# MarineRoboticsGroup/mac

Hardware: AMD Instinct MI355X
Metric: frank_wolfe_iters_per_sec (higher is better)
Workload: dtype f64; 1 GPU; configs[3]: ER N=100000 ~2M candidates, chain fixed, K=10%; N=100000, m_candidates=2001737, K=200173, fixed_edges=99999, fw_iters=209, parallelism=single GPU

## Files before the change

### include/machip.h

```cpp
#ifndef MACHIP_H
#define MACHIP_H

#include <stdint.h>

#ifdef __cplusplus
extern "C" {
#endif

#define MACHIP_ABI_VERSION 19

typedef enum machip_status {
    MACHIP_OK = 0,
    MACHIP_NOT_CONVERGED = 1,
    MACHIP_DISCONNECTED = 2,
    MACHIP_BAD_ARG = 3,
    MACHIP_HIP_ERROR = 4,
    MACHIP_RCCL_ERROR = 5,
    MACHIP_NO_DEVICE = 6
} machip_status;

typedef struct machip_problem machip_problem;

typedef struct machip_solve_stats {
    int64_t lanczos_steps;
    int64_t spmv_total;
    int64_t vec_passes;
    int64_t restarts;
    int64_t nnz;
    int64_t support;
    double residual;
    double lnorm;
    double gpu_ms;
    double step_ms;
    int64_t steps_timed;
    int64_t steps_lowp;
    double drift;
} machip_solve_stats;

int machip_version(void);
int machip_sizeof_stats(void);
int machip_device_count(void);
const char* machip_last_error(void);

int machip_create(int device, int64_t n,
                  int64_t n_fixed, const int32_t* fi, const int32_t* fj, const double* fw,
                  int64_t m, const int32_t* ci, const int32_t* cj, const double* cw,
                  double min_selection_weight_tol, machip_problem** out);
void machip_destroy(machip_problem* p);

int machip_set_x(machip_problem* p, const double* x);
int machip_get_x(machip_problem* p, double* x);

int machip_assemble(machip_problem* p, int64_t* nnz_out);
int machip_get_laplacian(machip_problem* p, int32_t* indptr, int32_t* indices, double* data);

int machip_fiedler(machip_problem* p, double tol, int max_steps, const double* x0, int warm_start,
                   double* lambda2, double* v_out, double* X_out, int q,
                   machip_solve_stats* stats);

int machip_lowest_pairs(machip_problem* p, int q, double tol, int max_steps, const double* X0, int warm_start,
                        double* lambda_out, double* V_out, double* residual_out, int32_t* steps_out, int32_t* restarts_out,
                        int32_t* status_out, int32_t* reordered_out, int32_t* first_rank_out);
int machip_lowest_pairs_csr(int device, int64_t n, const int32_t* indptr, const int32_t* indices, const double* data,
                            int q, double tol, int max_steps, const double* X0, int warm_start,
                            double* lambda_out, double* V_out, double* residual_out, int32_t* steps_out, int32_t* restarts_out,
                            int32_t* status_out, int32_t* reordered_out, int32_t* first_rank_out);
int machip_lowest_pairs_time(machip_problem* p, int q, double* ms_out);
int machip_gradient_block(machip_problem* p, int q, const double* V, double* G_out);

int machip_set_start(machip_problem* p, const double* x0);

int machip_gradient(machip_problem* p, double* g_out);

int machip_lp_topk(machip_problem* p, int64_t k, double* s_out);

int machip_fw_step(machip_problem* p, int64_t k, int iter, double tol, int max_steps, int warm_start,
                   double* f, double* dual, double* gnorm, machip_solve_stats* stats);
int machip_fw_commit(machip_problem* p);
int machip_fw_run(machip_problem* p, int64_t k, int first_iter, int max_iters, double gap_tol, double grad_tol, double tol,
                  int max_steps, int warm_start, double* upper_inout, double* f_traj, double* dual_traj, double* gnorm_traj,
                  machip_solve_stats* stats, int* modes, int* iters_done);

int machip_round_nearest(machip_problem* p, int64_t k, int decimals, double* rounded_out);

int machip_fiedler_csr(int device, int64_t n, const int32_t* indptr, const int32_t* indices,
                       const double* data, double tol, int max_steps, const double* x0,
// ... 102 lines not shown
```

### mac_amd/_lib.py

```python
from __future__ import annotations

import ctypes as C
import os

import numpy as np

_HERE = os.path.dirname(os.path.abspath(__file__))
LIB_PATH = os.environ.get("MACHIP_LIB") or os.path.join(_HERE, "libmachip.so")

OK, NOT_CONVERGED, DISCONNECTED, BAD_ARG, HIP_ERROR, RCCL_ERROR, NO_DEVICE = range(7)
STATUS_NAMES = ["OK", "NOT_CONVERGED", "DISCONNECTED", "BAD_ARG", "HIP_ERROR", "RCCL_ERROR", "NO_DEVICE"]


class MachipError(RuntimeError):
    def __init__(self, status, msg):
        super().__init__(f"libmachip: {STATUS_NAMES[status] if 0 <= status < 7 else status}: {msg}")
        self.status = status


class NotConverged(MachipError):
    pass


class Disconnected(MachipError):
    """lambda_2 ~ 0 (the reference fails with SuperLU 'Factor is exactly singular')."""


class SolveStats(C.Structure):
    _fields_ = [("lanczos_steps", C.c_int64), ("spmv_total", C.c_int64), ("vec_passes", C.c_int64),
                ("restarts", C.c_int64), ("nnz", C.c_int64), ("support", C.c_int64),
                ("residual", C.c_double), ("lnorm", C.c_double), ("gpu_ms", C.c_double),
                ("step_ms", C.c_double), ("steps_timed", C.c_int64), ("steps_lowp", C.c_int64), ("drift", C.c_double)]

    def asdict(self):
        return {k: getattr(self, k) for k, _ in self._fields_}


_i32p = C.POINTER(C.c_int32)
_f64p = C.POINTER(C.c_double)
_lib = None

_PAIRS_TAIL = [_f64p, _f64p, _f64p, _i32p, _i32p, _i32p, C.POINTER(C.c_int32), C.POINTER(C.c_int32)]
PAIRS_CHUNK = 16

SIGNATURES = {
    "machip_version": (C.c_int, []),
    "machip_sizeof_stats": (C.c_int, []),
    "machip_device_count": (C.c_int, []),
    "machip_last_error": (C.c_char_p, []),
    "machip_create": (C.c_int, [C.c_int, C.c_int64, C.c_int64, _i32p, _i32p, _f64p, C.c_int64, _i32p, _i32p,
                                _f64p, C.c_double, C.POINTER(C.c_void_p)]),
    "machip_destroy": (None, [C.c_void_p]),
    "machip_set_x": (C.c_int, [C.c_void_p, _f64p]),
    "machip_get_x": (C.c_int, [C.c_void_p, _f64p]),
    "machip_assemble": (C.c_int, [C.c_void_p, C.POINTER(C.c_int64)]),
    "machip_get_laplacian": (C.c_int, [C.c_void_p, _i32p, _i32p, _f64p]),
    "machip_fiedler": (C.c_int, [C.c_void_p, C.c_double, C.c_int, _f64p, C.c_int, _f64p, _f64p, _f64p, C.c_int,
                                 C.POINTER(SolveStats)]),
    "machip_lowest_pairs": (C.c_int, [C.c_void_p, C.c_int, C.c_double, C.c_int, _f64p, C.c_int] + _PAIRS_TAIL),
    "machip_lowest_pairs_csr": (C.c_int, [C.c_int, C.c_int64, _i32p, _i32p, _f64p, C.c_int, C.c_double, C.c_int, _f64p, C.c_int] + _PAIRS_TAIL),
    "machip_lowest_pairs_time": (C.c_int, [C.c_void_p, C.c_int, _f64p]),
    "machip_gradient_block": (C.c_int, [C.c_void_p, C.c_int, _f64p, _f64p]),
    "machip_set_start": (C.c_int, [C.c_void_p, _f64p]),
    "machip_gradient": (C.c_int, [C.c_void_p, _f64p]),
    "machip_lp_topk": (C.c_int, [C.c_void_p, C.c_int64, _f64p]),
    "machip_fw_step": (C.c_int, [C.c_void_p, C.c_int64, C.c_int, C.c_double, C.c_int, C.c_int, _f64p, _f64p,
                                 _f64p, C.POINTER(SolveStats)]),
    "machip_fw_commit": (C.c_int, [C.c_void_p]),
    "machip_fw_run": (C.c_int, [C.c_void_p, C.c_int64, C.c_int, C.c_int, C.c_double, C.c_double, C.c_double, C.c_int, C.c_int, _f64p, _f64p,
                                _f64p, _f64p, C.POINTER(SolveStats), C.POINTER(C.c_int), C.POINTER(C.c_int)]),
    "machip_round_nearest": (C.c_int, [C.c_void_p, C.c_int64, C.c_int, _f64p]),
    "machip_fiedler_csr": (C.c_int, [C.c_int, C.c_int64, _i32p, _i32p, _f64p, C.c_double, C.c_int, _f64p, _f64p,
                                     _f64p, _f64p, C.c_int, C.POINTER(SolveStats)]),
    "machip_spmv": (C.c_int, [C.c_void_p, _f64p, _f64p, C.c_int]),
    "machip_landscape": (C.c_int, [C.c_void_p, C.c_int, _f64p]),
    "machip_profile_spmv": (C.c_int, [C.c_void_p, C.c_int, _f64p, _f64p]),
    "machip_comm_unique_id": (C.c_int, [C.c_void_p]),
    "machip_comm_init": (C.c_int, [C.c_void_p, C.c_int, C.c_int, C.c_void_p]),
    "machip_comm_init_local": (C.c_int, [C.POINTER(C.c_void_p), C.c_int]),
    "machip_selftest_watchdog": (C.c_int, [C.c_int, C.c_int]),
    "machip_peer_access": (C.c_int, [C.c_int, C.c_int]),
    "machip_ipc_blob_bytes": (C.c_int, []),
    "machip_ipc_export": (C.c_int, [C.c_void_p, C.c_void_p, C.c_int]),
    "machip_comm_init_ipc": (C.c_int, [C.c_void_p, C.c_int, C.c_int, C.c_void_p, C.c_double]),
    "machip_comm_close_ipc": (C.c_int, [C.c_void_p]),
    "machip_comm_mode": (C.c_int, [C.c_void_p]),
    "machip_shard_plan": (C.c_int, [C.c_int64, C.c_int, C.c_int, C.POINTER(C.c_int64), C.POINTER(C.c_int64), C.POINTER(C.c_int64)]),
    "machip_eval_batch": (C.c_int, [C.c_void_p, C.c_int, _f64p, C.c_double, C.c_int, _f64p, C.POINTER(C.c_int)]),
# ... 169 lines not shown
        h = C.c_void_p()
        check(lib.machip_create(int(device), self.n, len(fw), p_i32(fi), p_i32(fj), p_f64(fw), self.m,
                                p_i32(ci), p_i32(cj), p_f64(cw), float(min_selection_weight_tol), C.byref(h)))
        self._h = h
        self._lib = lib
        self.stats = SolveStats()

    def close(self):
        if getattr(self, "_h", None):
            self._lib.machip_destroy(self._h)
            self._h = None

    def __del__(self):
        try:
            self.close()
        except Exception:
            pass

    def set_x(self, x):
        x = f64(x)
        assert x.shape == (self.m,)
        check(self._lib.machip_set_x(self._h, p_f64(x)))

    def get_x(self):
        x = np.empty(self.m)
        check(self._lib.machip_get_x(self._h, p_f64(x)))
        return x

    def assemble(self):
        nnz = C.c_int64()
        check(self._lib.machip_assemble(self._h, C.byref(nnz)))
        return int(nnz.value)

    def laplacian_csr(self):
        nnz = self.assemble()
        indptr = np.empty(self.n + 1, dtype=np.int32)
        indices = np.empty(nnz, dtype=np.int32)
        data = np.empty(nnz)
        check(self._lib.machip_get_laplacian(self._h, p_i32(indptr), p_i32(indices), p_f64(data)))
        return indptr, indices, data

    def spmv(self, v, variant=0):
        v = f64(v)
        y = np.empty(self.n)
        check(self._lib.machip_spmv(self._h, p_f64(v), p_f64(y), int(variant)))
        return y

    def landscape(self, sweeps=3):
        u = np.empty(self.n)
        check(self._lib.machip_landscape(self._h, int(sweeps), p_f64(u)))
        return u

    def fiedler(self, tol=1e-8, max_steps=0, x0=None, warm_start=False, want_vec=True, q=0):
        lam = C.c_double()
        v = np.empty(self.n) if want_vec else None
        X = np.empty((q, self.n)) if q else None
        x0a = f64(x0) if x0 is not None else None
        st = self._lib.machip_fiedler(self._h, float(tol), int(max_steps), p_f64(x0a), int(bool(warm_start)),
                                      C.byref(lam), p_f64(v), p_f64(X), int(q), C.byref(self.stats))
        check(st)
        return lam.value, v, (X.T if X is not None else None)

    def lowest_pairs(self, q=4, tol=1e-8, max_steps=0, X0=None, warm_start=False, raise_on_cap=False):
        X0 = None if X0 is None else np.asfortranarray(X0, dtype=np.float64)
        assert X0 is None or X0.shape == (self.n, q)
        return _pairs_call(lambda *tail: self._lib.machip_lowest_pairs(self._h, int(q), float(tol), int(max_steps), p_f64(X0),
# ... 500 lines not shown
```

### mac_amd/csrc/kernels.h

```cpp
#pragma once
#include <algorithm>

#include "common.h"

namespace machip {

template <typename T>
struct CsrViewT {
    int n;
    const int* rowptr;
    const int* col;
    const T* val;
};
using CsrView = CsrViewT<double>;

struct PatternView {
    int n;
    const int* prow;
    const int* pcol;
    const int* pk;
    const double* pw;
};

struct LanState {
// ... 42 lines not shown
        const int b = P.prow[r], e = P.prow[r + 1];
        int c = 0, sc = 0;
        for (int p = b + lane; p < e; p += G) {
            const int k = P.pk[p];
            const bool cand = k >= 0;
            const bool act = cand ? x_bit(xbits, k) : true;
            c += act;
            sc += (cand && act);
        }
        c = group_sum_i<G>(c);
        sc = group_sum_i<G>(sc);
        if (lane == 0) {
            cnt[r] = c + 1;
            local += c + 1;
            supp += sc;
            mx = max(mx, c + 1);
        }
    }
    const int tot = block_sum_i(local, sm);
    const int stot = block_sum_i(supp, sm);
#pragma unroll
    for (int o = 32; o > 0; o >>= 1) mx = max(mx, __shfl_xor(mx, o, kWave));
    __syncthreads();
    if ((threadIdx.x & 63) == 0) sm[threadIdx.x >> 6] = mx;
    __syncthreads();
    if (threadIdx.x == 0) {
        blk_sum[blockIdx.x] = tot;
        blk_sum[kAsmGrid + blockIdx.x] = stot;
        const int longest = max(max(sm[0], sm[1]), max(sm[2], sm[3]));
        blk_sum[2 * kAsmGrid + blockIdx.x] = longest;
        if (hsum) {
            hsum[blockIdx.x] = tot; hsum[kAsmGrid + blockIdx.x] = stot; hsum[2 * kAsmGrid + blockIdx.x] = longest;
        }
    }
}

struct PanSpec {
    int NP = 0;
    int C = 1;
    int band = 0;
    int* ps = nullptr;
    double* bd = nullptr;
    int* bpk = nullptr;
    int* ovf = nullptr;
};

template <int G>
__global__ __launch_bounds__(kBlock) void k_asm_fill(PatternView P, const unsigned int* __restrict__ xbits, const double* __restrict__ x,
                                                     int rows_per_block,
                                                     const int* __restrict__ cnt,
                                                     const int* __restrict__ blk_sum,
                                                     int* __restrict__ rowptr, int* __restrict__ col,
                                                     double* __restrict__ val,
                                                     double* __restrict__ blk_lnorm, PanSpec S = PanSpec()) {
    extern __shared__ __attribute__((aligned(16))) char smem_raw[];
    int* s_off = reinterpret_cast<int*>(smem_raw);
    __shared__ int sm_i[4];
    __shared__ double sm_d[4];
    __shared__ int s_chunk[kBlock];
    constexpr int GPB = kBlock / G;
    const int tid = threadIdx.x;
    const int lane = tid % G, g = tid / G;
    const int r0 = blockIdx.x * rows_per_block;
    const int r1 = min(P.n, r0 + rows_per_block);
    const int nr = max(0, r1 - r0);

// ... 1144 lines not shown
        st->prefix = s_prefix; st->kk = need; st->cnt_eq = eq; st->T = T; st->k = k;
        for (int i = 0; i < 7; ++i) st->ticket[i] = 0;
        st->ticket[7] = (unsigned int)s_done;
    }
    if (k <= 0) { if (tid == 0) st->tie_limit = prefer_high ? 0x7fffffffffffffffll : -1; return; }
    if (need >= eq) { if (tid == 0) st->tie_limit = prefer_high ? -1 : 0x7fffffffffffffffll; return; }
    long long runs = 0;
    for (long base = 0; base < m; base += 1024) {
        const long ii = base + tid;
        const long i = prefer_high ? m - 1 - ii : ii;
        const bool is = ii < m && f64_key(g[i]) == T;
        const unsigned long long bal = __ballot(is);
        __syncthreads();
        if (ln == 0) s_cnt[wv] = __popcll(bal);
        __syncthreads();
        int before = 0, tot = 0;
        for (int q = 0; q < 16; ++q) { if (q < wv) before += s_cnt[q]; tot += s_cnt[q]; }
        if (runs + tot >= need) {
            const int rank = before + __popcll(bal & ((1ull << ln) - 1ull));
            if (is && runs + rank + 1 == need) s_found = i;
            __syncthreads();
            if (tid == 0) st->tie_limit = s_found;
            return;
        }
        runs += tot;
    }
    if (tid == 0) st->tie_limit = prefer_high ? -1 : 0x7fffffffffffffffll;
}

__global__ __launch_bounds__(kBlock) void k_fw_final(const double* __restrict__ g, const double* __restrict__ x,
                                                     long m, const SelState* __restrict__ st, double gamma,
                                                     double* __restrict__ x_next, double* __restrict__ s_out,
                                                     double* __restrict__ part ,
                                                     double tol = 0.0, unsigned long long* __restrict__ xbits_next = nullptr) {
#pragma clang fp contract(off)
    __shared__ double sm[4];
    const unsigned long long T = st->T;
    const long long lim = st->tie_limit;
    const bool none = st->k <= 0;
    double d = 0.0, q = 0.0;
    for (long i = (long)blockIdx.x * kBlock + threadIdx.x; i < m; i += (long)gridDim.x * kBlock) {
        const double gi = g[i];
        const unsigned long long key = f64_key(gi);
        const double s = (!none && (key > T || (key == T && (long long)i <= lim))) ? 1.0 : 0.0;
        if (s_out) s_out[i] = s;
        if (x) {
            const double xi = x[i];
            const double diff = s - xi;
            d += gi * diff;
            q += gi * gi;
            if (x_next) {
                const double step = gamma * diff;
                const double xn = xi + step;
                x_next[i] = xn;
                if (xbits_next) {
                    const unsigned long long bal = __ballot(xn > tol);
                    if ((threadIdx.x & 63) == 0) xbits_next[i >> 6] = bal;
                }
            }
        }
    }
    d = block_sum(d, sm);
    q = block_sum(q, sm);
    if (threadIdx.x == 0) { part[blockIdx.x] = d; part[kMaxGrid + blockIdx.x] = q; }
}

__global__ __launch_bounds__(kBlock) void k_round_keys(const double* __restrict__ x, long m, double f,
                                                       double* __restrict__ r) {
#pragma clang fp contract(off)
    for (long i = (long)blockIdx.x * kBlock + threadIdx.x; i < m; i += (long)gridDim.x * kBlock) {
        const double t = x[i] * f;
        r[i] = rint(t) / f;
    }
}
__global__ __launch_bounds__(kBlock) void k_tie_keys(const double* __restrict__ r, const double* __restrict__ cw,
                                                     long m, const SelState* __restrict__ st1,
                                                     double* __restrict__ keys2) {
    const unsigned long long T = st1->T;
    for (long i = (long)blockIdx.x * kBlock + threadIdx.x; i < m; i += (long)gridDim.x * kBlock)
        keys2[i] = f64_key(r[i]) == T ? cw[i] : -__builtin_huge_val();
}
__global__ __launch_bounds__(kBlock) void k_round_mark(const double* __restrict__ r, const double* __restrict__ keys2,
                                                       long m, const SelState* __restrict__ st1,
                                                       const SelState* __restrict__ st2, int two_level,
                                                       double* __restrict__ out) {
    const unsigned long long T1 = st1->T;
    const bool none = st1->k <= 0;
    for (long i = (long)blockIdx.x * kBlock + threadIdx.x; i < m; i += (long)gridDim.x * kBlock) {
        const unsigned long long k1 = f64_key(r[i]);
        bool sel = false;
// ... 63 lines not shown
```

### mac_amd/csrc/mac.h

```cpp
#pragma once
#include <rccl/rccl.h>

#include <algorithm>
#include <cmath>
#include <condition_variable>
#include <memory>

#include "solver.h"

struct machip_problem;

namespace machip {

inline bool completed(int st) { return st == MACHIP_OK || st == MACHIP_NOT_CONVERGED || st == MACHIP_DISCONNECTED; }

struct LocalGroup {
    int nranks = 0;
    std::vector<double*> g;
    std::vector<machip_problem*> members;
    ShardGroup sg;
    bool shard_eig = false;
    int lead_status = MACHIP_OK;
    double lead_lam = 0.0;
    machip_solve_stats lead_stats{};
// ... 11 lines not shown
        std::unique_lock<std::mutex> lk(mu);
        if (broken) return false;
        const unsigned long gen = generation;
        if (++waiting == nranks) { waiting = 0; ++generation; cv.notify_all(); return true; }
        cv.wait(lk, [&] { return generation != gen || broken; });
        return !broken;
    }
    void abort() {
        std::lock_guard<std::mutex> lk(mu);
        broken = true;
        cv.notify_all();
    }
};

}

struct machip_problem {
    int device = 0;
    hipStream_t stream = nullptr;
    int n = 0;
    long m = 0, m_pad = 0;
    double tol_sel = 1e-10;
    int *prow = nullptr, *pcol = nullptr, *pk = nullptr;
    double* pw = nullptr;
    long P = 0;
    int asm_G = 16, asm_rpb = 1, asm_grid = 1;
    int *ci = nullptr, *cj = nullptr;
    double* cw = nullptr;
    double *x = nullptr, *x_next = nullptr, *g = nullptr, *s = nullptr, *scratch_m = nullptr;
    int *cnt = nullptr, *blk_sum = nullptr, *rowptr = nullptr, *col = nullptr;
    double *val = nullptr, *blk_lnorm = nullptr;
    unsigned long long *xb = nullptr, *xb_next = nullptr;
    bool xb_valid = false, xb_next_valid = false;
    long nnz = 0, support = 0;
    int maxlen = 0;
    double lnorm = 0.0;
    bool assembled = false, have_vec = false, csr_only = false;
    bool band_dups_ok = true;
    unsigned int* hist = nullptr;
    machip::SelState* sel = nullptr;
    double* part_fw = nullptr;
    int* h_int = nullptr;
    double* h_dbl = nullptr;
    int* d_hint = nullptr;
    double* d_hdbl = nullptr;
    machip::Solver sol;
    ncclComm_t comm = nullptr;
    std::shared_ptr<machip::LocalGroup> lgroup;
    bool first_collective_pending = false;
    hipEvent_t ev_g0 = nullptr, ev_g1 = nullptr, ev_g2 = nullptr;
    bool ev_g_valid = false;
    std::unique_ptr<machip::IpcGroup> ipcg;
    int rank = 0, nranks = 1;
    bool is_lane = false, lane_fw_ready = false;
    std::vector<machip_problem*> lanes;
    unsigned long start_version = 0;
    unsigned long seen_start_version = ~0ul;

    machip::CsrView csr() const { return machip::CsrView{n, rowptr, col, val}; }
    machip::PatternView pattern() const { return machip::PatternView{n, prow, pcol, pk, pw}; }
};

namespace machip {

inline std::mutex g_csr_mu;
inline machip_problem* g_csr_cache = nullptr;

struct Slot { int col, k; double w; };

inline int build_pattern(machip_problem* p, int64_t nf, const int32_t* fi, const int32_t* fj, const double* fw,
                         int64_t m, const int32_t* ci, const int32_t* cj, const double* cw) {
    const Options& opt = p->sol.opt;
    const int n = p->n;
    std::vector<long> deg((size_t)n + 1, 0);
    auto chk = [&](int a, int b) { return a >= 0 && a < n && b >= 0 && b < n; };
    for (int64_t e = 0; e < nf; ++e) {
        if (!chk(fi[e], fj[e])) return fail(MACHIP_BAD_ARG, "fixed edge endpoint out of range");
        if (fi[e] != fj[e]) { deg[(size_t)fi[e]]++; deg[(size_t)fj[e]]++; }
    }
    for (int64_t e = 0; e < m; ++e) {
        if (!chk(ci[e], cj[e])) return fail(MACHIP_BAD_ARG, "candidate edge endpoint out of range");
        if (ci[e] != cj[e]) { deg[(size_t)ci[e]]++; deg[(size_t)cj[e]]++; }
    }
    std::vector<long> off((size_t)n + 1, 0);
    for (int r = 0; r < n; ++r) off[(size_t)r + 1] = off[(size_t)r] + deg[(size_t)r];
    std::vector<Slot> slots((size_t)off[(size_t)n]);
    std::vector<long> cur(off.begin(), off.end() - 1);
    for (int64_t e = 0; e < nf; ++e) {
        const int a = fi[e], b = fj[e];
        if (a == b) continue;
        slots[(size_t)cur[(size_t)a]++] = Slot{b, -1, fw[e]};
        slots[(size_t)cur[(size_t)b]++] = Slot{a, -1, fw[e]};
    }
    for (int64_t e = 0; e < m; ++e) {
        const int a = ci[e], b = cj[e];
        if (a == b) continue;
        slots[(size_t)cur[(size_t)a]++] = Slot{b, (int)e, cw[e]};
        slots[(size_t)cur[(size_t)b]++] = Slot{a, (int)e, cw[e]};
    }
    std::vector<int> prow((size_t)n + 1, 0);
    std::vector<int> pcol, pk;
    std::vector<double> pw;
    pcol.reserve(slots.size()); pk.reserve(slots.size()); pw.reserve(slots.size());
    for (int r = 0; r < n; ++r) {
        Slot* b = slots.data() + off[(size_t)r];
        Slot* e = slots.data() + off[(size_t)r + 1];
        std::sort(b, e, [](const Slot& x, const Slot& y) {
            if (x.col != y.col) return x.col < y.col;
            return x.k < y.k;
        });
        for (Slot* q = b; q < e; ++q) {
            if (q->k < 0 && !pcol.empty() && (long)pcol.size() > prow[(size_t)r] && pcol.back() == q->col &&
                pk.back() < 0) {
                pw.back() += q->w;
            } else {
                pcol.push_back(q->col); pk.push_back(q->k); pw.push_back(q->w);
            }
        }
        if (pcol.size() > 2000000000ull) return fail(MACHIP_BAD_ARG, "pattern exceeds int32 indexing");
        {
            int band_slots = 0;
            for (size_t q = (size_t)prow[(size_t)r]; q < pcol.size(); ++q) band_slots += (pcol[q] == r - 1 || pcol[q] == r + 1);
            if (band_slots > 7) p->band_dups_ok = false;
        }
        prow[(size_t)r + 1] = (int)pcol.size();
    }
    p->P = (long)pcol.size();
    ST_TRY(dev_alloc(&p->prow, (size_t)n + 1));
    ST_TRY(dev_alloc(&p->pcol, (size_t)p->P)); ST_TRY(dev_alloc(&p->pk, (size_t)p->P)); ST_TRY(dev_alloc(&p->pw, (size_t)p->P));
    HIP_TRY(hipMemcpyAsync(p->prow, prow.data(), sizeof(int) * ((size_t)n + 1), hipMemcpyHostToDevice, p->stream));
    if (p->P) {
        HIP_TRY(hipMemcpyAsync(p->pcol, pcol.data(), sizeof(int) * (size_t)p->P, hipMemcpyHostToDevice, p->stream));
        HIP_TRY(hipMemcpyAsync(p->pk, pk.data(), sizeof(int) * (size_t)p->P, hipMemcpyHostToDevice, p->stream));
        HIP_TRY(hipMemcpyAsync(p->pw, pw.data(), sizeof(double) * (size_t)p->P, hipMemcpyHostToDevice, p->stream));
    }
    HIP_TRY(hipStreamSynchronize(p->stream));
    const double mean = n ? (double)p->P / n : 1.0;
    int G = 4;
    while (G < 64 && G < mean * 0.75) G <<= 1;
    p->asm_G = OPT(asm_g, G);
    const int gpb = kBlock / p->asm_G;
    long nblk = std::min<long>(std::min(kAsmGrid, std::max(1, OPT(asm_maxgrid, kAsmGrid))), ((long)n + gpb - 1) / gpb);
    if (nblk < 1) nblk = 1;
    long rpb = ((long)n + nblk - 1) / nblk;
    rpb = (rpb + gpb - 1) / gpb * gpb;
    p->asm_rpb = (int)rpb;
    p->asm_grid = (int)(((long)n + rpb - 1) / rpb);
    if (p->asm_grid < 1) p->asm_grid = 1;
    if ((rpb + 1) * (long)sizeof(int) > 64 * 1024)
        return fail(MACHIP_BAD_ARG, "num_nodes above the supported 16.7 million (row-offset scan of the assembly kernel)");
    return MACHIP_OK;
}

template <int G>
void launch_asm(machip_problem* p, const PanSpec& S) {
    const PatternView P = p->pattern();
    const unsigned int* xb32 = reinterpret_cast<const unsigned int*>(p->xb);
    k_asm_count<G><<<p->asm_grid, kBlock, 0, p->stream>>>(P, xb32, p->asm_rpb, p->cnt, p->blk_sum, p->d_hint);
    const size_t lds = sizeof(int) * ((size_t)p->asm_rpb + 1);
    k_asm_fill<G><<<p->asm_grid, kBlock, lds, p->stream>>>(P, xb32, p->x, p->asm_rpb, p->cnt, p->blk_sum,
                                                           p->rowptr, p->col, p->val, p->d_hdbl, S);
}

inline int assemble(machip_problem* p) {
    if (p->csr_only) return fail(MACHIP_BAD_ARG, "handle wraps a caller CSR; nothing to assemble");
    PanSpec S;
    ST_TRY(p->sol.pan_spec_prepare(&S));
    if (!p->xb_valid) {
        const int grid = std::max(1, (int)std::min<long>(kMaxGrid, (p->m + kBlock - 1) / kBlock));
        k_x_bits<<<grid, kBlock, 0, p->stream>>>(p->x, p->m, p->tol_sel, p->xb);
        p->xb_valid = true;
    }
    switch (p->asm_G) {
        case 4: launch_asm<4>(p, S); break;
        case 8: launch_asm<8>(p, S); break;
        case 16: launch_asm<16>(p, S); break;
        case 32: launch_asm<32>(p, S); break;
        default: launch_asm<64>(p, S); break;
    }
    HIP_TRY(hipGetLastError());
    const int gb = p->asm_grid;
    HIP_TRY(hipStreamSynchronize(p->stream));
    long nnz = 0, supp = 0;
    int maxlen = 0;
    double ln = 0.0;
    for (int b = 0; b < gb; ++b) {
        nnz += p->h_int[b]; supp += p->h_int[kAsmGrid + b]; maxlen = std::max(maxlen, p->h_int[2 * kAsmGrid + b]);
        ln = std::max(ln, p->h_dbl[b]);
    }
    p->nnz = nnz; p->support = supp / 2; p->lnorm = ln; p->maxlen = maxlen;
    p->assembled = true;
    return MACHIP_OK;
}

inline int alloc_common(machip_problem* p, int vbudget_mb = 0) {
    ST_TRY(p->sol.init(p->n, p->stream, vbudget_mb));
    HIP_TRY(hipHostMalloc((void**)&p->h_int, sizeof(int) * 3 * kAsmGrid, hipHostMallocMapped));
    HIP_TRY(hipHostMalloc((void**)&p->h_dbl, sizeof(double) * std::max(4 * kMaxGrid, kAsmGrid), hipHostMallocMapped));
    HIP_TRY(hipHostGetDevicePointer((void**)&p->d_hint, p->h_int, 0));
    HIP_TRY(hipHostGetDevicePointer((void**)&p->d_hdbl, p->h_dbl, 0));
    return MACHIP_OK;
}

inline int alloc_assembly(machip_problem* p) {
    const size_t cap = (size_t)p->P + (size_t)p->n + 8;
    ST_TRY(dev_alloc(&p->cnt, (size_t)p->n + 1)); ST_TRY(dev_alloc(&p->blk_sum, 3 * kAsmGrid));
    ST_TRY(dev_alloc(&p->rowptr, (size_t)p->n + 1)); ST_TRY(dev_alloc(&p->col, cap)); ST_TRY(dev_alloc(&p->val, cap));
    ST_TRY(dev_alloc(&p->blk_lnorm, kAsmGrid));
    ST_TRY(dev_alloc(&p->xb, (size_t)p->m / 64 + 2)); ST_TRY(dev_alloc(&p->xb_next, (size_t)p->m / 64 + 2));
    p->sol.csr_cap = cap;
    return MACHIP_OK;
}

inline int alloc_fw(machip_problem* p) {
    const size_t mp = (size_t)p->m + 64 * 8;
    if (!p->x_next) ST_TRY(dev_alloc(&p->x_next, mp));
    if (!p->g) ST_TRY(dev_alloc(&p->g, mp));
    if (!p->s) ST_TRY(dev_alloc(&p->s, mp));
    return MACHIP_OK;
}
inline int alloc_fw_select(machip_problem* p) {
    if (!p->hist) ST_TRY(dev_alloc(&p->hist, (6 + kSelRep) * kBins));
    if (!p->sel) ST_TRY(dev_alloc(&p->sel, 2));
    if (!p->part_fw) ST_TRY(dev_alloc(&p->part_fw, 2 * kMaxGrid));
// ... 22 lines not shown
        HIP_TRY(hipStreamSynchronize(p->stream));
        p->sol.have_start = true;
        ++p->start_version;
    }
    machip_solve_stats local;
    memset(&local, 0, sizeof(local));
    p->sol.maxlen_hint = p->maxlen;
    p->sol.support_hint = (p->csr_only && !p->sol.chain_like) ? -1 : p->support;
    p->sol.start_guess = x0 != nullptr;
    const int st = p->sol.solve(p->csr(), p->nnz, p->lnorm, tol, max_steps, (x0 == nullptr && warm_start) ? 1 : 0,
                                kAuto, lambda2, &local);
    p->sol.start_guess = false;
    local.support = p->support;
    if (stats) *stats = local;
    p->have_vec = completed(st);
    return st;
}

inline void set_option(machip_problem* p, int id, long v) {
    p->sol.opt.v[id] = v;
    for (machip_problem* q : p->lanes) q->sol.opt.v[id] = v;
}

inline void ipc_abort(machip_problem* p) {
    k_ipc_abort<<<1, 64, 0, p->stream>>>(p->ipcg->view);
    (void)hipStreamSynchronize(p->stream);
}

inline void destroy_handle(machip_problem* p) {
    for (machip_problem* q : p->lanes) destroy_handle(q);
    p->lanes.clear();
    (void)hipSetDevice(p->device);
    if (p->stream) (void)hipStreamSynchronize(p->stream);
    if (p->is_lane) { p->prow = p->pcol = p->pk = nullptr; p->pw = nullptr; p->ci = p->cj = nullptr; p->cw = nullptr; }
    if (p->comm) (void)ncclCommDestroy(p->comm);
    if (p->lgroup) p->lgroup->abort();
    if (p->ipcg) {
        if (!p->ipcg->clean_exit) ipc_abort(p);
        p->sol.ipc = nullptr;
        p->ipcg.reset();
    }
    p->sol.destroy();
    void* ptrs[] = {p->prow, p->pcol, p->pk, p->pw, p->ci, p->cj, p->cw, p->x, p->x_next, p->g, p->s, p->scratch_m, p->cnt,
                    p->blk_sum, p->rowptr, p->col, p->val, p->blk_lnorm, p->xb, p->xb_next, p->hist, p->sel, p->part_fw};
    for (void* q : ptrs) if (q) (void)hipFree(q);
    for (hipEvent_t e : {p->ev_g0, p->ev_g1, p->ev_g2}) if (e) (void)hipEventDestroy(e);
    if (p->h_int) (void)hipHostFree(p->h_int);
    if (p->h_dbl) (void)hipHostFree(p->h_dbl);
    if (p->stream) (void)hipStreamDestroy(p->stream);
    delete p;
}

inline int create_handle(int device, int64_t n, int64_t n_fixed, const int32_t* fi, const int32_t* fj, const double* fw, int64_t m,
                         const int32_t* ci, const int32_t* cj, const double* cw, double min_sel_tol, machip_problem** out) {
    machip_problem* p = new machip_problem();
    p->device = device; p->n = (int)n; p->m = p->m_pad = (long)m; p->tol_sel = min_sel_tol;
    auto body = [&]() -> int {
        HIP_TRY(hipStreamCreateWithFlags(&p->stream, hipStreamNonBlocking));
        ST_TRY(build_pattern(p, n_fixed, fi, fj, fw, m, ci, cj, cw));
        const size_t mp = (size_t)m + 64 * 8;
        ST_TRY(dev_alloc(&p->ci, mp)); ST_TRY(dev_alloc(&p->cj, mp)); ST_TRY(dev_alloc(&p->cw, mp));
        ST_TRY(dev_alloc(&p->x, mp)); ST_TRY(alloc_fw(p));
        if (m) {
            HIP_TRY(hipMemcpyAsync(p->ci, ci, sizeof(int) * (size_t)m, hipMemcpyHostToDevice, p->stream));
            HIP_TRY(hipMemcpyAsync(p->cj, cj, sizeof(int) * (size_t)m, hipMemcpyHostToDevice, p->stream));
            HIP_TRY(hipMemcpyAsync(p->cw, cw, sizeof(double) * (size_t)m, hipMemcpyHostToDevice, p->stream));
        }
        HIP_TRY(hipMemsetAsync(p->x, 0, sizeof(double) * mp, p->stream));
        HIP_TRY(hipMemsetAsync(p->g, 0, sizeof(double) * mp, p->stream));
        HIP_TRY(hipStreamSynchronize(p->stream));
        ST_TRY(alloc_assembly(p));
        ST_TRY(alloc_fw_select(p));
        ST_TRY(alloc_common(p));
        p->sol.pat = p->pattern();
        p->sol.pan_allowed = p->band_dups_ok;
        {
            std::vector<char> has((size_t)n, 0);
// ... 233 lines not shown
```

### mac_amd/csrc/mac_fw.h

```cpp
#pragma once
#include "mac_comm.h"

namespace machip {

inline int lp_topk(machip_problem* p, int64_t k, double* s_out) {
    ST_TRY(select_topk(p, (long)k));
    const int grid = (int)std::min<long>(kMaxGrid, (p->m + kBlock - 1) / kBlock);
    k_fw_final<<<std::max(grid, 1), kBlock, 0, p->stream>>>(p->g, nullptr, p->m, p->sel, 0.0, nullptr, p->s, p->part_fw);
    if (s_out) HIP_TRY(hipMemcpyAsync(s_out, p->s, sizeof(double) * (size_t)p->m, hipMemcpyDeviceToHost, p->stream));
    HIP_TRY(hipStreamSynchronize(p->stream));
    return MACHIP_OK;
}

inline int fw_step(machip_problem* p, int64_t k, int iter, double tol, int max_steps, int warm_start,
                   double* f, double* dual, double* gnorm, machip_solve_stats* stats) {
    GroupGuard guard{p};
    HIP_TRY(hipSetDevice(p->device));
    ST_TRY(assemble(p));
    double lam = 0.0;
    const int grid = std::max(1, (int)std::min<long>(kMaxGrid, (p->m + kBlock - 1) / kBlock));
    const double gamma = 2.0 / ((double)iter + 2.0);
    int epi_status = MACHIP_OK;
    auto epilogue = [&](bool speculative) {
        bool fused = false;
        int st = compute_gradient(p, speculative, (long)k, &fused);
        if (st == MACHIP_OK) st = select_topk(p, (long)k, fused);
        if (st == MACHIP_OK) {
            k_fw_final<<<grid, kBlock, 0, p->stream>>>(p->g, p->x, p->m, p->sel, gamma, p->x_next, nullptr, p->d_hdbl, p->tol_sel, p->xb_next);
            p->xb_next_valid = true;
            if (hipGetLastError() != hipSuccess) st = fail(MACHIP_HIP_ERROR, "k_fw_final launch failed");
        }
        epi_status = st;
    };
    bool done = false;
    if (p->lgroup && p->lgroup->shard_eig) {
        const int st = group_fiedler(p, tol, max_steps, warm_start, &lam, stats);
        if (st != MACHIP_OK) { guard.ok = completed(st); return st; }
    } else {
        const bool spec = p->nranks <= 1 && p->sol.opt.get(kOpt_spec_epilogue, 1) != 0;
        if (spec) p->sol.after_check = [&] { epilogue(true); };
        const int st = run_fiedler(p, tol, max_steps, nullptr, warm_start, &lam, stats);
        p->sol.after_check = nullptr;
        if (st != MACHIP_OK) { guard.ok = completed(st); return st; }
        done = spec && p->sol.hook_seq == p->sol.final_check_seq && epi_status == MACHIP_OK;
    }
    if (!done) {
        epilogue(false);
        if (epi_status != MACHIP_OK) return epi_status;
        HIP_TRY(hipStreamSynchronize(p->stream));
    }
    if (p->ipcg) ST_TRY(p->sol.ipc_check_err("gradient exchange"));
    double d = 0.0, q2 = 0.0;
    for (int b = 0; b < grid; ++b) { d += p->h_dbl[b]; q2 += p->h_dbl[kMaxGrid + b]; }
    *f = lam;
    *dual = lam + d;
    *gnorm = std::sqrt(q2);
    guard.ok = true;
    return MACHIP_OK;
}

inline void fw_commit(machip_problem* p) {
    std::swap(p->x, p->x_next);
    std::swap(p->xb, p->xb_next);
    p->xb_valid = p->xb_next_valid; p->xb_next_valid = false;
    p->assembled = false;
}

template <class OnIter>
int fw_loop(machip_problem* p, int64_t k, int first_iter, int max_iters, double gap_tol, double grad_tol, double tol, int max_steps,
            int warm_start, machip_solve_stats* stats, double* upper_inout, int* iters_done, OnIter&& on_iter) {
    double u = *upper_inout;
    int done = 0, rc = MACHIP_OK;
    for (int i = 0; i < max_iters; ++i) {
        double f = 0.0, dual = 0.0, gn = 0.0;
        if (stats) memset(stats, 0, sizeof(*stats));
        rc = fw_step(p, k, first_iter + i, tol, max_steps, (warm_start && (first_iter + i) > 0) ? 1 : 0, &f, &dual, &gn, stats);
        if (rc != MACHIP_OK) break;
        u = std::min(u, dual);
        on_iter(i, f, dual, gn, stats);
        done = i + 1;
        if (gn < grad_tol) break;
        if ((u - f) < gap_tol * std::fabs(f)) break;
        fw_commit(p);
    }
    *upper_inout = u; *iters_done = done;
    return rc;
}

inline int decimals_ok(int decimals) { return decimals > 15 ? fail(MACHIP_BAD_ARG, "decimals must be <= 15") : (int)MACHIP_OK; }
inline int round_nearest(machip_problem* p, int64_t k, int decimals, double* rounded_out) {
    ST_TRY(decimals_ok(decimals));
    const long m = p->m;
    if (m == 0) return MACHIP_OK;
    if (!p->scratch_m) ST_TRY(dev_alloc(&p->scratch_m, (size_t)m + 64));
    const int grid = std::max(1, (int)std::min<long>(kMaxGrid, (m + kBlock - 1) / kBlock));
    double* r = p->s;
    const bool tb = decimals >= 0;
// ... 22 lines not shown
```

### mac_amd/csrc/mac_lanes.h

```cpp
#pragma once
#include <atomic>
#include <limits>
#include <thread>

#include "mac_fw.h"

namespace machip {

inline int create_lane_stream(const Options& opt, int device, hipStream_t* out) {
    if (OPT(lane_queues, 0) == 0) {
        hipDeviceProp_t prop;
        if (hipGetDeviceProperties(&prop, device) == hipSuccess && prop.multiProcessorCount > 0) {
            const int words = (prop.multiProcessorCount + 31) / 32;
            std::vector<uint32_t> mask((size_t)words, 0xffffffffu);
            if (prop.multiProcessorCount % 32) mask.back() = (1u << (prop.multiProcessorCount % 32)) - 1u;
            if (hipExtStreamCreateWithCUMask(out, (uint32_t)words, mask.data()) == hipSuccess) return MACHIP_OK;
            (void)hipGetLastError();
        }
    }
    HIP_TRY(hipStreamCreateWithFlags(out, hipStreamNonBlocking));
    return MACHIP_OK;
}

inline int make_lane(machip_problem* p, machip_problem** out) {
    machip_problem* q = new machip_problem();
    q->is_lane = true;
    q->device = p->device; q->n = p->n; q->m = p->m; q->m_pad = p->m; q->tol_sel = p->tol_sel;
    q->prow = p->prow; q->pcol = p->pcol; q->pk = p->pk; q->pw = p->pw; q->P = p->P;
    q->asm_G = p->asm_G; q->asm_rpb = p->asm_rpb; q->asm_grid = p->asm_grid;
    q->ci = p->ci; q->cj = p->cj; q->cw = p->cw;
    auto body = [&]() -> int {
        ST_TRY(create_lane_stream(p->sol.opt, q->device, &q->stream));
        ST_TRY(dev_alloc(&q->x, (size_t)q->m + 64));
        ST_TRY(alloc_assembly(q));
        const Options& opt = p->sol.opt;
        q->sol.opt = opt;
        ST_TRY(alloc_common(q, std::max(16, OPT(lane_vbudget_mb, std::max(16, OPT(vbudget_mb, 4096) / 8)))));
        q->sol.pat = q->pattern();
        q->sol.pan_allowed = p->sol.pan_allowed;
        q->sol.chain_like = p->sol.chain_like; q->sol.chain_edges = p->sol.chain_edges;
        return MACHIP_OK;
    };
    const int st = body();
    if (st != MACHIP_OK) { destroy_handle(q); return st; }
    *out = q;
    return MACHIP_OK;
}

inline int ensure_lane_fw(machip_problem* q) {
    if (q->lane_fw_ready) return MACHIP_OK;
    const size_t mp = (size_t)q->m + 64 * 8;
    ST_TRY(alloc_fw(q)); ST_TRY(alloc_fw_select(q));
    HIP_TRY(hipMemsetAsync(q->g, 0, sizeof(double) * mp, q->stream));
    HIP_TRY(hipStreamSynchronize(q->stream));
    q->lane_fw_ready = true;
    return MACHIP_OK;
}

inline int prepare_lanes(machip_problem* p, int B, bool fw, int* nl_out) {
    const bool small = p->sol.chain_like && persist_fits(p->n, std::max(0l, (long)p->P - 2 * p->sol.chain_edges));
    const Options& opt = p->sol.opt;
// ... 101 lines not shown
```

### mac_amd/csrc/machip.hip

```cpp
#include <climits>

#include "mac_lanes.h"
#include "esp.h"
#include "esp_free.h"
#include "esp_tree.h"
#include "esp_select.h"
#include "esp_relax.h"
#include "esp_exchange.h"
#include "esp_exchange_edge.h"
#include "eig_exchange.h"
#include "eig_routes.h"

namespace machip {
thread_local std::string g_err;
}
using namespace machip;

extern "C" {

int machip_version(void) { return MACHIP_ABI_VERSION; }
int machip_sizeof_stats(void) { return (int)sizeof(machip_solve_stats); }

int machip_device_count(void) {
    int c = 0;
// ... 13 lines not shown
    if (n_fixed < 0 || m < 0 || m > 2000000000ll) return fail(MACHIP_BAD_ARG, "bad edge counts");
    if ((n_fixed && (!fi || !fj || !fw)) || (m && (!ci || !cj || !cw))) return fail(MACHIP_BAD_ARG, "NULL edge array");
    if (n_fixed + m < n - 1) return fail(MACHIP_BAD_ARG, "fewer than n-1 edges: no spanning tree possible");
    if ((double)(n_fixed + m) > 0.5 * (double)n * (double)(n - 1)) return fail(MACHIP_BAD_ARG, "more edges than the complete graph");
    if (machip_device_count() <= 0) return fail(MACHIP_NO_DEVICE, "no HIP device visible");
    HIP_TRY(hipSetDevice(device));
    return create_handle(device, n, n_fixed, fi, fj, fw, m, ci, cj, cw, min_sel_tol, out);
}

void machip_destroy(machip_problem* p) { if (p) destroy_handle(p); }

int machip_set_x(machip_problem* p, const double* x) {
    if (!p || !x || p->csr_only) return fail(MACHIP_BAD_ARG, "machip_set_x: bad handle or NULL x");
    HIP_TRY(hipSetDevice(p->device));
    HIP_TRY(hipMemcpyAsync(p->x, x, sizeof(double) * (size_t)p->m, hipMemcpyHostToDevice, p->stream));
    HIP_TRY(hipStreamSynchronize(p->stream));
    p->assembled = false; p->xb_valid = false;
    return MACHIP_OK;
}

int machip_get_x(machip_problem* p, double* x) {
    if (!p || !x || p->csr_only) return fail(MACHIP_BAD_ARG, "machip_get_x: bad handle or NULL x");
    HIP_TRY(hipSetDevice(p->device));
    HIP_TRY(hipMemcpyAsync(x, p->x, sizeof(double) * (size_t)p->m, hipMemcpyDeviceToHost, p->stream));
    HIP_TRY(hipStreamSynchronize(p->stream));
    return MACHIP_OK;
}

int machip_assemble(machip_problem* p, int64_t* nnz_out) {
    if (!p) return fail(MACHIP_BAD_ARG, "NULL handle");
    HIP_TRY(hipSetDevice(p->device));
    ST_TRY(assemble(p));
    if (nnz_out) *nnz_out = p->nnz;
    return MACHIP_OK;
}

int machip_get_laplacian(machip_problem* p, int32_t* indptr, int32_t* indices, double* data) {
    if (!p || !indptr || !indices || !data) return fail(MACHIP_BAD_ARG, "NULL argument");
    HIP_TRY(hipSetDevice(p->device));
    if (!p->assembled) ST_TRY(assemble(p));
    HIP_TRY(hipMemcpyAsync(indptr, p->rowptr, sizeof(int) * ((size_t)p->n + 1), hipMemcpyDeviceToHost, p->stream));
    HIP_TRY(hipMemcpyAsync(indices, p->col, sizeof(int) * (size_t)p->nnz, hipMemcpyDeviceToHost, p->stream));
    HIP_TRY(hipMemcpyAsync(data, p->val, sizeof(double) * (size_t)p->nnz, hipMemcpyDeviceToHost, p->stream));
    HIP_TRY(hipStreamSynchronize(p->stream));
    return MACHIP_OK;
}

int machip_fiedler(machip_problem* p, double tol, int max_steps, const double* x0, int warm_start,
                   double* lambda2, double* v_out, double* X_out, int q, machip_solve_stats* stats) {
    if (!p || !lambda2) return fail(MACHIP_BAD_ARG, "NULL argument");
    if (X_out && (q < 1 || q > 4)) return fail(MACHIP_BAD_ARG, "q must be in [1,4]");
    HIP_TRY(hipSetDevice(p->device));
    const int st = run_fiedler(p, tol, max_steps, x0, warm_start, lambda2, stats);
    if (!completed(st)) return st;
    const std::string keep = g_err;
    if (v_out) {
        HIP_TRY(hipMemcpyAsync(v_out, p->sol.yvec, sizeof(double) * (size_t)p->n, hipMemcpyDeviceToHost, p->stream));
        HIP_TRY(hipStreamSynchronize(p->stream));
    }
    if (X_out) ST_TRY(p->sol.ritz_block(q, X_out));
    g_err = keep;
    return st;
}

int machip_set_start(machip_problem* p, const double* x0) {
    if (!p || !x0) return fail(MACHIP_BAD_ARG, "NULL argument");
// ... 602 lines not shown
```

### mac_amd/csrc/options.h

```cpp
#pragma once
#include <climits>
#include <cstdlib>
#include <cstring>
#include <mutex>
#include <string>

namespace machip {

#define MACHIP_OPTION_LIST(X)                                                                                                      \
                                                                                                          \
    X(solver) X(graph) X(debug) X(chunk) X(chunk_near) X(sched) X(near_x10) X(trigger_pct) X(classic_n) X(persist) X(pchunk)      \
    X(spec_epilogue) X(spec_slack_pct) X(f32_switch_e9) X(tailless) X(stream) X(stream_trigger_pct) X(stream_retry_pct) X(stream_look) X(stream_margin) X(stream_window) X(stream_far) X(start_land) X(start_pow) X(start_floor_e6) X(start_land_pr_permille) X(start_land_min_mean10)                                                                \
                                                                        \
    X(spmv) X(g) X(unroll) X(block) X(maxgrid) X(defer) X(tpr) X(ell)                                                              \
                                                                                                            \
    X(panel) X(panel_min_n) X(panel_min_mean10) X(panel_multi_min_mean10) X(panel_np) X(panel_nb) X(panel_b2) X(panel_g2)         \
    X(panel_cells) X(panel_maxcells) X(panel_band) X(panel_u) X(panel_u_amp) X(pan32) X(pan32_switch_e9) X(panel_ops) X(panel_rev)                                                                               \
                                                                                                 \
    X(woodbury) X(wb_max) X(wb_hard) X(wb_lane_max) X(exact_big) X(exact_switch) X(gj_look_min) X(lob_density_pct) X(lob_chunk)   \
    X(lob_patience) X(lob_small_s) X(lob_fuse)                                                                                     \
     \
    X(sel_small) X(sel_fuse) X(asm_g) X(asm_maxgrid) X(vbudget_mb) X(vcap) X(lanes) X(lane_vbudget_mb) X(lane_queues) X(shard_eig) X(ipc_panel) \
    X(rccl_timeout_s)                                                                                                              \
               \
    X(esp_free_split)                                                                                                              \
       \
    X(esp_xch_lds_kb) X(esp_xch_max_mb) X(esp_xch_profile)                                                                         \
                                                       \
    X(eig_xch_max_mb)                                                                                                              \
                                                                                        \
    X(eig_xch_free_swaps)                                                                                                          \
                                                                                                            \
    X(eig_free_rows) X(eig_free_split)                                                                                             \
                                    \
    X(pairs_vcap)

enum OptId {
#define X(n) kOpt_##n,
    MACHIP_OPTION_LIST(X)
#undef X
    kNumOpts
};

constexpr long kOptAuto = LONG_MIN;

inline const char* const* option_names() {
    static const char* const names[] = {
#define X(n) #n,
        MACHIP_OPTION_LIST(X)
#undef X
        nullptr};
    return names;
}
inline int option_id(const char* name) {
    if (!name) return -1;
// ... 48 lines not shown
```

Measured before the change: 131.7 iter/s.

## Maintain Laplacian row counts incrementally from selection-bit flips in FW step

The Frank-Wolfe final kernel now compares the new selection bitmask with the previous one. For each flipped candidate it atomically adjusts the per-row nonzero counts of both endpoints, and a small per-block reduction kernel then rebuilds the block sums. The next assembly can skip the full k_asm_count pass over the pattern. This adds atomics, a per-row fixed-edge count array and cross-call state tracking. It is enabled by default only on single-GPU runs with at least about 2M pattern slots.

```diff
diff --git a/include/machip.h b/include/machip.h
--- a/include/machip.h
+++ b/include/machip.h
@@ -7,7 +7,7 @@
 extern "C" {
 #endif
 
-#define MACHIP_ABI_VERSION 19
+#define MACHIP_ABI_VERSION 20
 
 typedef enum machip_status {
     MACHIP_OK = 0,
@@ -52,6 +52,7 @@
 int machip_get_x(machip_problem* p, double* x);
 
 int machip_assemble(machip_problem* p, int64_t* nnz_out);
+int machip_assembly_info(machip_problem* p, int64_t* nnz_out, int64_t* support_out, int* maxlen_out);
 int machip_get_laplacian(machip_problem* p, int32_t* indptr, int32_t* indices, double* data);
 
 int machip_fiedler(machip_problem* p, double tol, int max_steps, const double* x0, int warm_start,
diff --git a/mac_amd/_lib.py b/mac_amd/_lib.py
--- a/mac_amd/_lib.py
+++ b/mac_amd/_lib.py
@@ -54,6 +54,7 @@
     "machip_set_x": (C.c_int, [C.c_void_p, _f64p]),
     "machip_get_x": (C.c_int, [C.c_void_p, _f64p]),
     "machip_assemble": (C.c_int, [C.c_void_p, C.POINTER(C.c_int64)]),
+    "machip_assembly_info": (C.c_int, [C.c_void_p, C.POINTER(C.c_int64), C.POINTER(C.c_int64), C.POINTER(C.c_int)]),
     "machip_get_laplacian": (C.c_int, [C.c_void_p, _i32p, _i32p, _f64p]),
     "machip_fiedler": (C.c_int, [C.c_void_p, C.c_double, C.c_int, _f64p, C.c_int, _f64p, _f64p, _f64p, C.c_int,
                                  C.POINTER(SolveStats)]),
@@ -289,6 +290,11 @@
         check(self._lib.machip_assemble(self._h, C.byref(nnz)))
         return int(nnz.value)
 
+    def assembly_info(self):
+        nnz, supp, mx = C.c_int64(), C.c_int64(), C.c_int()
+        check(self._lib.machip_assembly_info(self._h, C.byref(nnz), C.byref(supp), C.byref(mx)))
+        return int(nnz.value), int(supp.value), int(mx.value)
+
     def laplacian_csr(self):
         nnz = self.assemble()
         indptr = np.empty(self.n + 1, dtype=np.int32)
diff --git a/mac_amd/csrc/kernels.h b/mac_amd/csrc/kernels.h
--- a/mac_amd/csrc/kernels.h
+++ b/mac_amd/csrc/kernels.h
@@ -98,6 +98,29 @@
         if (hsum) {
             hsum[blockIdx.x] = tot; hsum[kAsmGrid + blockIdx.x] = stot; hsum[2 * kAsmGrid + blockIdx.x] = longest;
         }
+    }
+}
+
+__global__ __launch_bounds__(kBlock) void k_asm_blocks(int n, int rows_per_block, int nblocks, const int* __restrict__ cnt,
+                                                       const int* __restrict__ nfix, int* __restrict__ blk_sum, int* __restrict__ hsum) {
+    const int b = blockIdx.x * (kBlock / kWave) + (threadIdx.x >> 6);
+    if (b >= nblocks) return;
+    const int r0 = b * rows_per_block;
+    const int r1 = min(n, r0 + rows_per_block);
+    int tot = 0, stot = 0, mx = 0;
+    for (int r = r0 + (int)(threadIdx.x & 63); r < r1; r += kWave) {
+        const int c = cnt[r];
+        tot += c;
+        stot += c - 1 - nfix[r];
+        mx = max(mx, c);
+    }
+    tot = wave_sum_i(tot);
+    stot = wave_sum_i(stot);
+#pragma unroll
+    for (int o = 32; o > 0; o >>= 1) mx = max(mx, __shfl_xor(mx, o, kWave));
+    if ((threadIdx.x & 63) == 0) {
+        blk_sum[b] = tot; blk_sum[kAsmGrid + b] = stot; blk_sum[2 * kAsmGrid + b] = mx;
+        hsum[b] = tot; hsum[kAsmGrid + b] = stot; hsum[2 * kAsmGrid + b] = mx;
     }
 }
 
@@ -1308,7 +1331,9 @@
                                                      long m, const SelState* __restrict__ st, double gamma,
                                                      double* __restrict__ x_next, double* __restrict__ s_out,
                                                      double* __restrict__ part ,
-                                                     double tol = 0.0, unsigned long long* __restrict__ xbits_next = nullptr) {
+                                                     double tol = 0.0, unsigned long long* xbits_next = nullptr,
+                                                     const unsigned long long* xbits_cnt = nullptr, int* __restrict__ cnt = nullptr,
+                                                     const int* __restrict__ ci = nullptr, const int* __restrict__ cj = nullptr) {
 #pragma clang fp contract(off)
     __shared__ double sm[4];
     const unsigned long long T = st->T;
@@ -1316,6 +1341,8 @@
     const bool none = st->k <= 0;
     double d = 0.0, q = 0.0;
     for (long i = (long)blockIdx.x * kBlock + threadIdx.x; i < m; i += (long)gridDim.x * kBlock) {
+        unsigned long long oldw = 0;
+        if (cnt && (threadIdx.x & 63) == 0) oldw = xbits_cnt[i >> 6];
         const double gi = g[i];
         const unsigned long long key = f64_key(gi);
         const double s = (!none && (key > T || (key == T && (long long)i <= lim))) ? 1.0 : 0.0;
@@ -1331,7 +1358,13 @@
                 x_next[i] = xn;
                 if (xbits_next) {
                     const unsigned long long bal = __ballot(xn > tol);
+                    const unsigned long long flip = cnt ? (__shfl(oldw, 0, kWave) ^ bal) : 0ull;
                     if ((threadIdx.x & 63) == 0) xbits_next[i >> 6] = bal;
+                    if ((flip >> (threadIdx.x & 63)) & 1ull) {
+                        const int dlt = ((bal >> (threadIdx.x & 63)) & 1ull) ? 1 : -1;
+                        atomicAdd(&cnt[ci[i]], dlt);
+                        atomicAdd(&cnt[cj[i]], dlt);
+                    }
                 }
             }
         }
diff --git a/mac_amd/csrc/mac.h b/mac_amd/csrc/mac.h
--- a/mac_amd/csrc/mac.h
+++ b/mac_amd/csrc/mac.h
@@ -67,6 +67,9 @@
     double *val = nullptr, *blk_lnorm = nullptr;
     unsigned long long *xb = nullptr, *xb_next = nullptr;
     bool xb_valid = false, xb_next_valid = false;
+    int cnt_of = 0;
+    int* nfix = nullptr;
+    bool two_slots = true;
     long nnz = 0, support = 0;
     int maxlen = 0;
     double lnorm = 0.0;
@@ -129,12 +132,12 @@
     }
     for (int64_t e = 0; e < m; ++e) {
         const int a = ci[e], b = cj[e];
-        if (a == b) continue;
+        if (a == b) { p->two_slots = false; continue; }
         slots[(size_t)cur[(size_t)a]++] = Slot{b, (int)e, cw[e]};
         slots[(size_t)cur[(size_t)b]++] = Slot{a, (int)e, cw[e]};
     }
     std::vector<int> prow((size_t)n + 1, 0);
-    std::vector<int> pcol, pk;
+    std::vector<int> pcol, pk, nfix((size_t)n, 0);
     std::vector<double> pw;
     pcol.reserve(slots.size()); pk.reserve(slots.size()); pw.reserve(slots.size());
     for (int r = 0; r < n; ++r) {
@@ -158,12 +161,14 @@
             for (size_t q = (size_t)prow[(size_t)r]; q < pcol.size(); ++q) band_slots += (pcol[q] == r - 1 || pcol[q] == r + 1);
             if (band_slots > 7) p->band_dups_ok = false;
         }
+        for (size_t q = (size_t)prow[(size_t)r]; q < pk.size(); ++q) nfix[(size_t)r] += pk[q] < 0;
         prow[(size_t)r + 1] = (int)pcol.size();
     }
     p->P = (long)pcol.size();
-    ST_TRY(dev_alloc(&p->prow, (size_t)n + 1));
+    ST_TRY(dev_alloc(&p->prow, (size_t)n + 1)); ST_TRY(dev_alloc(&p->nfix, (size_t)n));
     ST_TRY(dev_alloc(&p->pcol, (size_t)p->P)); ST_TRY(dev_alloc(&p->pk, (size_t)p->P)); ST_TRY(dev_alloc(&p->pw, (size_t)p->P));
     HIP_TRY(hipMemcpyAsync(p->prow, prow.data(), sizeof(int) * ((size_t)n + 1), hipMemcpyHostToDevice, p->stream));
+    HIP_TRY(hipMemcpyAsync(p->nfix, nfix.data(), sizeof(int) * (size_t)n, hipMemcpyHostToDevice, p->stream));
     if (p->P) {
         HIP_TRY(hipMemcpyAsync(p->pcol, pcol.data(), sizeof(int) * (size_t)p->P, hipMemcpyHostToDevice, p->stream));
         HIP_TRY(hipMemcpyAsync(p->pk, pk.data(), sizeof(int) * (size_t)p->P, hipMemcpyHostToDevice, p->stream));
@@ -187,11 +192,17 @@
     return MACHIP_OK;
 }
 
+constexpr long kAsmDeltaMinSlots = 2l << 20;
+inline bool asm_delta_on(const machip_problem* p) {
+    const long v = p->sol.opt.v[kOpt_asm_delta];
+    return v == kOptAuto ? p->P >= kAsmDeltaMinSlots : v != 0;
+}
+
 template <int G>
-void launch_asm(machip_problem* p, const PanSpec& S) {
+void launch_asm(machip_problem* p, const PanSpec& S, bool count) {
     const PatternView P = p->pattern();
     const unsigned int* xb32 = reinterpret_cast<const unsigned int*>(p->xb);
-    k_asm_count<G><<<p->asm_grid, kBlock, 0, p->stream>>>(P, xb32, p->asm_rpb, p->cnt, p->blk_sum, p->d_hint);
+    if (count) k_asm_count<G><<<p->asm_grid, kBlock, 0, p->stream>>>(P, xb32, p->asm_rpb, p->cnt, p->blk_sum, p->d_hint);
     const size_t lds = sizeof(int) * ((size_t)p->asm_rpb + 1);
     k_asm_fill<G><<<p->asm_grid, kBlock, lds, p->stream>>>(P, xb32, p->x, p->asm_rpb, p->cnt, p->blk_sum,
                                                            p->rowptr, p->col, p->val, p->d_hdbl, S);
@@ -205,14 +216,17 @@
         const int grid = std::max(1, (int)std::min<long>(kMaxGrid, (p->m + kBlock - 1) / kBlock));
         k_x_bits<<<grid, kBlock, 0, p->stream>>>(p->x, p->m, p->tol_sel, p->xb);
         p->xb_valid = true;
-    }
+        p->cnt_of = 0;
+    }
+    const bool count = !(p->cnt_of == 1 && asm_delta_on(p));
     switch (p->asm_G) {
-        case 4: launch_asm<4>(p, S); break;
-        case 8: launch_asm<8>(p, S); break;
-        case 16: launch_asm<16>(p, S); break;
-        case 32: launch_asm<32>(p, S); break;
-        default: launch_asm<64>(p, S); break;
-    }
+        case 4: launch_asm<4>(p, S, count); break;
+        case 8: launch_asm<8>(p, S, count); break;
+        case 16: launch_asm<16>(p, S, count); break;
+        case 32: launch_asm<32>(p, S, count); break;
+        default: launch_asm<64>(p, S, count); break;
+    }
+    p->cnt_of = 0;
     HIP_TRY(hipGetLastError());
     const int gb = p->asm_grid;
     HIP_TRY(hipStreamSynchronize(p->stream));
@@ -225,6 +239,7 @@
     }
     p->nnz = nnz; p->support = supp / 2; p->lnorm = ln; p->maxlen = maxlen;
     p->assembled = true;
+    p->cnt_of = 1;
     return MACHIP_OK;
 }
 
@@ -313,7 +328,7 @@
     p->lanes.clear();
     (void)hipSetDevice(p->device);
     if (p->stream) (void)hipStreamSynchronize(p->stream);
-    if (p->is_lane) { p->prow = p->pcol = p->pk = nullptr; p->pw = nullptr; p->ci = p->cj = nullptr; p->cw = nullptr; }
+    if (p->is_lane) { p->prow = p->pcol = p->pk = p->nfix = nullptr; p->pw = nullptr; p->ci = p->cj = nullptr; p->cw = nullptr; }
     if (p->comm) (void)ncclCommDestroy(p->comm);
     if (p->lgroup) p->lgroup->abort();
     if (p->ipcg) {
@@ -323,7 +338,7 @@
     }
     p->sol.destroy();
     void* ptrs[] = {p->prow, p->pcol, p->pk, p->pw, p->ci, p->cj, p->cw, p->x, p->x_next, p->g, p->s, p->scratch_m, p->cnt,
-                    p->blk_sum, p->rowptr, p->col, p->val, p->blk_lnorm, p->xb, p->xb_next, p->hist, p->sel, p->part_fw};
+                    p->blk_sum, p->rowptr, p->col, p->val, p->blk_lnorm, p->xb, p->xb_next, p->hist, p->sel, p->part_fw, p->nfix};
     for (void* q : ptrs) if (q) (void)hipFree(q);
     for (hipEvent_t e : {p->ev_g0, p->ev_g1, p->ev_g2}) if (e) (void)hipEventDestroy(e);
     if (p->h_int) (void)hipHostFree(p->h_int);
diff --git a/mac_amd/csrc/mac_fw.h b/mac_amd/csrc/mac_fw.h
--- a/mac_amd/csrc/mac_fw.h
+++ b/mac_amd/csrc/mac_fw.h
@@ -26,7 +26,17 @@
         int st = compute_gradient(p, speculative, (long)k, &fused);
         if (st == MACHIP_OK) st = select_topk(p, (long)k, fused);
         if (st == MACHIP_OK) {
-            k_fw_final<<<grid, kBlock, 0, p->stream>>>(p->g, p->x, p->m, p->sel, gamma, p->x_next, nullptr, p->d_hdbl, p->tol_sel, p->xb_next);
+            const bool delta = p->cnt_of != 0 && p->two_slots && p->nranks <= 1 && !p->lgroup && !p->ipcg && asm_delta_on(p);
+            if (delta) {
+                k_fw_final<<<grid, kBlock, 0, p->stream>>>(p->g, p->x, p->m, p->sel, gamma, p->x_next, nullptr, p->d_hdbl, p->tol_sel, p->xb_next,
+                                                            p->cnt_of == 2 ? p->xb_next : p->xb, p->cnt, p->ci, p->cj);
+                k_asm_blocks<<<(p->asm_grid + kBlock / kWave - 1) / (kBlock / kWave), kBlock, 0, p->stream>>>(p->n, p->asm_rpb, p->asm_grid, p->cnt, p->nfix,
+                                                                                                             p->blk_sum, p->d_hint);
+                p->cnt_of = 2;
+            } else {
+                k_fw_final<<<grid, kBlock, 0, p->stream>>>(p->g, p->x, p->m, p->sel, gamma, p->x_next, nullptr, p->d_hdbl, p->tol_sel, p->xb_next);
+                p->cnt_of = 0;
+            }
             p->xb_next_valid = true;
             if (hipGetLastError() != hipSuccess) st = fail(MACHIP_HIP_ERROR, "k_fw_final launch failed");
         }
@@ -63,6 +73,7 @@
     std::swap(p->x, p->x_next);
     std::swap(p->xb, p->xb_next);
     p->xb_valid = p->xb_next_valid; p->xb_next_valid = false;
+    p->cnt_of = (p->cnt_of == 2 && p->xb_valid) ? 1 : 0;
     p->assembled = false;
 }
 
diff --git a/mac_amd/csrc/mac_lanes.h b/mac_amd/csrc/mac_lanes.h
--- a/mac_amd/csrc/mac_lanes.h
+++ b/mac_amd/csrc/mac_lanes.h
@@ -26,7 +26,7 @@
     machip_problem* q = new machip_problem();
     q->is_lane = true;
     q->device = p->device; q->n = p->n; q->m = p->m; q->m_pad = p->m; q->tol_sel = p->tol_sel;
-    q->prow = p->prow; q->pcol = p->pcol; q->pk = p->pk; q->pw = p->pw; q->P = p->P;
+    q->prow = p->prow; q->pcol = p->pcol; q->pk = p->pk; q->pw = p->pw; q->P = p->P; q->nfix = p->nfix; q->two_slots = p->two_slots;
     q->asm_G = p->asm_G; q->asm_rpb = p->asm_rpb; q->asm_grid = p->asm_grid;
     q->ci = p->ci; q->cj = p->cj; q->cw = p->cw;
     auto body = [&]() -> int {
diff --git a/mac_amd/csrc/machip.hip b/mac_amd/csrc/machip.hip
--- a/mac_amd/csrc/machip.hip
+++ b/mac_amd/csrc/machip.hip
@@ -69,6 +69,16 @@
     HIP_TRY(hipSetDevice(p->device));
     ST_TRY(assemble(p));
     if (nnz_out) *nnz_out = p->nnz;
+    return MACHIP_OK;
+}
+
+int machip_assembly_info(machip_problem* p, int64_t* nnz_out, int64_t* support_out, int* maxlen_out) {
+    if (!p || p->csr_only) return fail(MACHIP_BAD_ARG, "bad handle");
+    HIP_TRY(hipSetDevice(p->device));
+    if (!p->assembled) ST_TRY(assemble(p));
+    if (nnz_out) *nnz_out = p->nnz;
+    if (support_out) *support_out = p->support;
+    if (maxlen_out) *maxlen_out = p->maxlen;
     return MACHIP_OK;
 }
 
diff --git a/mac_amd/csrc/options.h b/mac_amd/csrc/options.h
--- a/mac_amd/csrc/options.h
+++ b/mac_amd/csrc/options.h
@@ -19,8 +19,8 @@
                                                                                                  \
     X(woodbury) X(wb_max) X(wb_hard) X(wb_lane_max) X(exact_big) X(exact_switch) X(gj_look_min) X(lob_density_pct) X(lob_chunk)   \
     X(lob_patience) X(lob_small_s) X(lob_fuse)                                                                                     \
-     \
-    X(sel_small) X(sel_fuse) X(asm_g) X(asm_maxgrid) X(vbudget_mb) X(vcap) X(lanes) X(lane_vbudget_mb) X(lane_queues) X(shard_eig) X(ipc_panel) \
+                              \
+    X(sel_small) X(sel_fuse) X(asm_delta) X(asm_g) X(asm_maxgrid) X(vbudget_mb) X(vcap) X(lanes) X(lane_vbudget_mb) X(lane_queues) X(shard_eig) X(ipc_panel) \
     X(rccl_timeout_s)                                                                                                              \
                \
     X(esp_free_split)                                                                                                              \
```

Result: slower. 129.9 iter/s (-1.4%).
